# haoningwu3639/StoryGen

Measured on AMD Instinct MI355X. Metric: UNet denoising steps/sec @512x512, 3 prior-frame ctx, bs=1, higher is better.
Workload: dtype f16; 1 GPU; BASELINE configs[1]: StoryGen denoising loop, 512x512 (64x64x4 latent), R=3 prior frames, CFG batch 3, DDIM, SD-1.5 UNet + attn3 (909M params, synthetic fp16 weights); stage=multi-image-condition, samples_per_gpu=1, parallelism=dp1 (one sample per GPU, final all-gather), hipgraph=True, dedup_identical_reference_samples=True, overlap_ref_pass_of_next_step=True, ref_ahead=1, warmup_run=5, split_graphs=False, stream_priority=False, ref_pass_on_cus=0, ref_pass_eager=False, paired_gemm_launches=True, paired_text_image_attention=False, groupnorm_stats_from_epilogues=True, fp16_block_stream=False

## Files before the change

storygen_amd/csrc/attention.hip:

```cpp
#include "attention_kernel.h"
#include <float.h>

using namespace sgattn;


static int attn_params(const sg_attn_desc* d, AttnParams& p, const char* who) {
    SG_REQUIRE(d != nullptr, "%s: null descriptor", who);
    SG_REQUIRE(d->q && d->k && d->vt && d->o, "%s: null q/k/vt/o", who);
    SG_REQUIRE(d->B > 0 && d->H > 0 && d->Nq > 0 && d->Nk > 0, "%s: bad shape", who);
    if (d->D != 40 && d->D != 80 && d->D != 160)
        return sg_set_error(SG_EUNSUP, "%s: head dim %d not in {40, 80, 160}", who, d->D);
    SG_REQUIRE(d->Nq <= (1 << 30) && d->Nk <= (1 << 30), "%s: Nq and Nk must not exceed 2^30", who);
    SG_REQUIRE(d->scale > 0.f && d->scale <= FLT_MAX, "%s: scale must be finite and > 0", who);
    SG_REQUIRE(d->kv_batches >= 0 && d->kv_batches <= d->B, "%s: kv_batches must be in [0, B]", who);
    SG_REQUIRE(d->kv_batches == 0 || 2 * (int64_t)d->kv_batches >= d->B, "%s: kv_batches must be 0 or at least B / 2", who);
    SG_REQUIRE(d->ldq % 8 == 0 && d->ldk % 8 == 0 && d->ldvt % 8 == 0 && d->ldo % 4 == 0, "%s: row strides", who);
    SG_REQUIRE(d->bsq % 8 == 0 && d->bsk % 8 == 0 && d->bsvt % 8 == 0 && d->bso % 4 == 0, "%s: batch strides", who);
    SG_REQUIRE(sg_aligned16(d->q) && sg_aligned16(d->k) && sg_aligned16(d->vt) && sg_aligned16(d->o), "%s: 16-byte alignment", who);
    const int64_t hd = (int64_t)d->H * d->D;
    SG_REQUIRE(d->ldq >= hd && d->ldk >= hd && d->ldo >= hd, "%s: token stride smaller than H*D", who);
    SG_REQUIRE(d->ldvt >= ((d->Nk + 7) & ~7), "%s: ldvt must cover Nk rounded up to 8 keys", who);
    SG_REQUIRE((int64_t)d->D * d->ldvt < (1ll << 31), "%s: VT head slab too large for 32-bit offsets", who);
    SG_REQUIRE(d->ldk < (1ll << 25), "%s: K tile (64 ldk) too large for 32-bit offsets", who);
    p = AttnParams{};
// ... 29 lines not shown
    if (lse) return attn_plan_grid(pl, d, SG_ATTN_LSE, 4, 3, who);
    const bool big = attn_big(d);
    const SgOptions& opt = sg_options();
    if (d->D == 40) {
        if (big && opt.attn_d40_general) return attn_plan_grid(pl, d, SG_ATTN_GENERAL, 4, 3, who);
        if (big && opt.attn_lean) return attn_plan_grid(pl, d, SG_ATTN_LEAN, 4, 3, who);
        return attn_plan_grid(pl, d, opt.attn_d40_loop == 1 ? SG_ATTN_SHARED_BODY : SG_ATTN_D40_LOOP, big ? 4 : 2, big ? 3 : 2, who);
    }
    if (d->D == 160 && opt.attn_d160 == 4 && d->Nq <= 256 && d->Nk > KVBLK && (long)sg_cdiv(d->Nq, 32) * d->H * d->B <= 256)
        return attn_plan_grid(pl, d, SG_ATTN_KSPLIT, 4, 1, who);
    return attn_plan_grid(pl, d, SG_ATTN_GENERAL, 4, 3, who);
}

static int attn_launch(const AttnParams& p, int D, const sg_attn_plan& pl, hipStream_t st) {
    const bool big = pl.waves == 4;
    switch (pl.family) {
    case SG_ATTN_LSE:
        if (D == 40) launch_attn<40, 4, 3, true, false, true>(p, st);
        else if (D == 80) launch_attn<80, 4, 3, true>(p, st);
        else launch_attn<160, 4, 3, true>(p, st);
        return SG_OK;
    case SG_ATTN_D40_LOOP: big ? launch_attn_d40<4, 3>(p, st) : launch_attn_d40<2, 2>(p, st); return SG_OK;
    case SG_ATTN_SHARED_BODY: big ? launch_attn<40, 4, 3>(p, st) : launch_attn<40, 2, 2>(p, st); return SG_OK;
    case SG_ATTN_LEAN: launch_attn<40, 4, 3, false, true>(p, st); return SG_OK;
    case SG_ATTN_KSPLIT: launch_attn_ksplit<160, 4>(p, st); return SG_OK;
    case SG_ATTN_GENERAL:
        if (D == 40) launch_attn<40, 4, 3, false, false, true>(p, st);
        else if (D == 80) launch_attn<80, 4, 3>(p, st);
        else launch_attn<160, 4, 3>(p, st);
        return SG_OK;
    }
    return sg_set_error(SG_EINVAL, "attention: internal: no kernel for plan family %d", pl.family);
}

static int attn_fwd(const sg_attn_desc* d, float* lse2, sg_stream_t stream) {
    const char* who = lse2 ? "sg_attn_fwd_lse_f16" : "sg_attn_fwd_f16";
    AttnParams p;
    sg_attn_plan pl;
    if (int rc = attn_params(d, p, "sg_attn_fwd_f16")) return rc;
    if (int rc = attn_plan(d, lse2 != nullptr, pl, "sg_attn_fwd_f16")) return rc;
    p.lse2 = lse2;
    if (int rc = attn_launch(p, d->D, pl, (hipStream_t)stream)) return rc;
    SG_CHECK_LAUNCH(who);
    return SG_OK;
}

extern "C" int sg_attn_fwd_f16(const sg_attn_desc* d, sg_stream_t stream) { return attn_fwd(d, nullptr, stream); }

extern "C" int sg_attn_fwd_plan(const sg_attn_desc* d, int32_t lse, sg_attn_plan* out) {
    SG_REQUIRE(out != nullptr, "sg_attn_fwd_plan: null plan");
    AttnParams p;
    if (int rc = attn_params(d, p, "sg_attn_fwd_plan")) return rc;
    return attn_plan(d, lse != 0, *out, "sg_attn_fwd_plan");
}

static int attn_pair_plan(const sg_attn_desc* d0, const sg_attn_desc* d1, sg_attn_pair_plan& pr, const char* who) {
    const SgOptions& opt = sg_options();
    const bool same = d0->D == d1->D && d0->B == d1->B && d0->H == d1->H && d0->Nq == d1->Nq;
    const bool defaults = !(d0->D == 40 && opt.attn_d40_loop == 1);
    pr = sg_attn_pair_plan{};
    if (!same || !defaults) {
        if (int rc = attn_plan(d0, false, pr.p0, who)) return rc;
        return attn_plan(d1, false, pr.p1, who);
    }
    const bool big = d0->D != 40 || attn_big(d0);
    const int family = d0->D == 40 ? SG_ATTN_D40_LOOP : SG_ATTN_GENERAL;
    if (int rc = attn_plan_grid(pr.p0, d0, family, big ? 4 : 2, big ? 3 : 2, who)) return rc;
    pr.p1 = pr.p0;
    SG_REQUIRE((int64_t)pr.p0.workgroups * 2 < (1ll << 31), "%s: the shared grid does not fit", who);
    pr.shared = 1;
    pr.first = d0->Nk >= d1->Nk ? 0 : 1;
    pr.workgroups = 2 * pr.p0.workgroups;
    return SG_OK;
}
// ... 39 lines not shown
```

storygen_amd/csrc/attention_kernel.h:

```cpp
#pragma once
#include "common.h"
#include <stdlib.h>
#include <type_traits>

namespace sgattn {


constexpr int KVBLK = 64;
constexpr float RESCALE_THR = 6.0f;

struct AttnParams {
    const f16* q; long ldq, bsq;
    const f16* k; long ldk, bsk;
    const f16* vt; long ldvt, bsvt;
    f16* o; long ldo, bso;
    int B, H, Nq, Nk, kv_batches, nqb;
    const f16* k2; long bsk2; const f16* vt2; long bsvt2; int Nk2, kv2;
    float scale_log2;
    float* lse2;
};

__device__ __forceinline__ void glds16(const f16* g, char* lds_wave_base) {
    __builtin_amdgcn_global_load_lds((const __attribute__((address_space(1))) void*)g,
                                     (__attribute__((address_space(3))) void*)lds_wave_base, 16, 0, 0);
// ... 4 lines not shown
}

template <int D>
__device__ __forceinline__ int kswz(int row) {
    return D == 40 ? 0 : (D == 80 ? ((row >> 3) & 1) : ((row >> 2) & 3));
}

constexpr int F40_KPAD = 2688;
constexpr int F40_ONES = 128;

template <int D, int NIMG>
constexpr int attn_smem_bytes() {
    return D == 40 ? F40_KPAD + NIMG * (KVBLK * D * 2 + D * 128 + F40_ONES) : NIMG * (KVBLK * D * 2 + D * 128) + (D % 16 == 0 ? 0 : 16);
}

template <int D, int NW, int S, bool LSE, bool LEAN = false, bool GENERAL = false, bool KSPLIT = false>
__device__ __forceinline__ void attn_fwd_body(const AttnParams& p, char* smem, const int block, const int nblocks) {
    constexpr int SUB = KSPLIT ? NW : 1;
    constexpr bool F40 = D == 40 && !GENERAL;
    constexpr int DC = D / 8;
    constexpr int NDK = (D + 15) / 16;
    constexpr int DT = (D + 31) / 32;
    constexpr int KROW = D * 2;
    constexpr int K_BYTES = KVBLK * KROW;
    constexpr int V_BYTES = D * 128;
    constexpr int K_SEG = K_BYTES / 1024, V_SEG = V_BYTES / 1024, NSEG = K_SEG + V_SEG;
    constexpr int TSTAGE = K_BYTES + V_BYTES + (F40 ? F40_ONES : 0);
    constexpr int STAGE = SUB * TSTAGE;
    constexpr int RING0 = F40 ? F40_KPAD : 0;
    constexpr int MAXL = (NSEG + NW - 1) / NW;
    constexpr int REM = NSEG % NW;
    static_assert(KSPLIT ? (S == 1 && !LSE && !(D == 40 && !GENERAL)) : (S == 2 || S == 3), "2 or 3 stages; key split: one stage of NW tiles");
    static_assert(!KSPLIT || NW * (8 + DT * 64) * 64 <= S * SUB * (KVBLK * D * 2 + D * 128), "the merge images of the waves fit the dead ring");
    static_assert((S - 1) * MAXL < 64, "vmcnt is a 6-bit counter");
    static_assert(RING0 + S * STAGE + (F40 || D % 16 == 0 ? 0 : 16) <= attn_smem_bytes<D, S * SUB>(), "LDS size");
    static_assert(!F40 || (32 * KROW + 16 <= F40_KPAD && F40_KPAD % 128 == 0), "K pad constants of both 32-key blocks");

    const int t = threadIdx.x, lane = t & 63, l31 = lane & 31, hi = lane >> 5;
    const int wave = __builtin_amdgcn_readfirstlane(t >> 6);
    const int work = xcd_remap(block, nblocks);
    const int bh = work / p.nqb, qb = work - bh * p.nqb;
    const int h = bh / p.B, b = bh - h * p.B;
    const int kvb = b < p.kv_batches ? b : b - (p.B - p.kv_batches);
    const bool short_row = kvb < p.kv2;
    const int Nk = short_row ? p.Nk2 : p.Nk;
    const int q0 = KSPLIT ? qb * 32 : (qb * NW + wave) * 32;
    const f16* Q = p.q + (long)b * p.bsq + (long)h * D;
    const f16* K = (short_row ? p.k2 + (long)kvb * p.bsk2 : p.k + (long)(kvb - p.kv2) * p.bsk) + (long)h * D;
    const f16* VT = (short_row ? p.vt2 + (long)kvb * p.bsvt2 : p.vt + (long)(kvb - p.kv2) * p.bsvt) + (long)h * D * p.ldvt;
// ... 22 lines not shown
            const int s = (g - K_SEG) * 64 + lane;
            const int d = s >> 3, cs = s & 7;
            row = d * (int)p.ldvt;
            col = (cs ^ ((d >> 1) & 7)) * 8;
        }
    };
    unsigned off[MAXL];
#pragma unroll
    for (int i = 0; i < MAXL; ++i) {
        const int g = i * NW + wave;
        int row, col;
        coords(g, row, col);
        off[i] = g < K_SEG ? (unsigned)(row * (int)p.ldk + col) : (unsigned)(row + col);
    }
    const int ntiles = (Nk + KVBLK - 1) / KVBLK;
    auto issue_tile = [&](int tile, char* base) __attribute__((always_inline)) {
        const int key0 = tile * KVBLK;
        if (key0 + KVBLK <= Nk) {
            const f16* Kt = K + (long)key0 * p.ldk;
            const f16* Vt = VT + key0;
#pragma unroll
            for (int i = 0; i < MAXL; ++i) {
                const int g = i * NW + wave;
                const f16* src = (g < K_SEG ? Kt : Vt) + off[i];
                if ((i + 1) * NW <= NSEG || g < NSEG) glds16(src, base + g * 1024);
            }
        } else {
#pragma unroll
            for (int i = 0; i < MAXL; ++i) {
                const int g = i * NW + wave;
                int row, col;
                coords(g, row, col);
                if (g < K_SEG) {
                    const int key = min(key0 + row, Nk - 1);
                    glds16(K + (long)key * p.ldk + col, base + g * 1024);
                } else if (g < NSEG) {
                    const int kc = min(key0 + col, nkp8 - 8);
                    glds16(VT + row + kc, base + g * 1024);
                }
            }
// ... 24 lines not shown

    f32x16 oacc[DT];
#pragma unroll
    for (int i = 0; i < DT; ++i)
#pragma unroll
        for (int r = 0; r < 16; ++r) oacc[i][r] = 0.f;
    float m_run = F40 ? 0.f : -INFINITY;
    float l_run = 0.f;

    const int ngroups = (ntiles + SUB - 1) / SUB;
#pragma unroll
    for (int s = 0; s < S - 1; ++s)
        if (s < ngroups) issue(s, s);

    const int prow = (l31 & ~12) | ((l31 & 4) << 1) | ((l31 & 8) >> 1);
    constexpr bool UNR = D == 40;
    int rt_stage = 0;
    for (int group0 = 0; group0 < ngroups; group0 += (UNR ? S : 1)) {
#pragma unroll
    for (int ustage = 0; ustage < (UNR ? S : 1); ++ustage) {
        const int group = group0 + ustage;
        const int stage = UNR ? ustage : rt_stage;
        if (group < ngroups) {
        if constexpr (KSPLIT) {
            if (group > 0) __builtin_amdgcn_s_barrier();
            issue(group, 0);
            wait_vmcnt<0>();
            __builtin_amdgcn_s_barrier();
        } else {
        if (S == 3 && group + 1 < ngroups) {
// ... 1 lines not shown
            else wait_vmcnt<(MAXL > 1 ? MAXL - 1 : 0)>();
        } else {
            wait_vmcnt<0>();
        }
        __builtin_amdgcn_s_barrier();
        if (group + S - 1 < ngroups) {
            int st = stage + S - 1;
            if (st >= S) st -= S;
            issue(group + S - 1, st);
        }
        }
#pragma unroll
      for (int subi = 0; subi < 1; ++subi) {
        const int sub = KSPLIT ? wave : subi;
        const int tile = group * SUB + sub;
        if (tile < ntiles) {
        const char* sK = smem + RING0 + stage * STAGE + sub * TSTAGE;
        const char* sV = sK + K_BYTES;

        f32x16 s[2];
        const f32x16 zero16 = {0.f, 0.f, 0.f, 0.f, 0.f, 0.f, 0.f, 0.f, 0.f, 0.f, 0.f, 0.f, 0.f, 0.f, 0.f, 0.f};
        constexpr bool KBATCH = NDK <= 5;
        if constexpr (KBATCH) {
            f16x8 kf[2][NDK];
            if constexpr (F40) {
                const char* k01 = sK + prow * KROW + hi * 16;
                const char* k2 = hi ? smem : sK + prow * KROW + 64;
#pragma unroll
                for (int kb = 0; kb < 2; ++kb) {
                    kf[kb][0] = *reinterpret_cast<const f16x8*>(k01 + kb * 32 * KROW);
                    kf[kb][1] = *reinterpret_cast<const f16x8*>(k01 + kb * 32 * KROW + 32);
                    kf[kb][2] = *reinterpret_cast<const f16x8*>(k2 + kb * 32 * KROW);
                }
            } else {
#pragma unroll
                for (int kb = 0; kb < 2; ++kb) {
                    const int row = kb * 32 + prow;
                    const char* krow = sK + row * KROW;
                    const int sw = kswz<D>(row);
#pragma unroll
                    for (int st = 0; st < NDK; ++st)
                        kf[kb][st] = *reinterpret_cast<const f16x8*>(krow + (((st * 2 + hi) ^ sw) << 4));
                }
            }
            __builtin_amdgcn_sched_barrier(0);
#pragma unroll
            for (int kb = 0; kb < 2; ++kb)
#pragma unroll
                for (int st = 0; st < NDK; ++st)
                    s[kb] = __builtin_amdgcn_mfma_f32_32x32x16_f16(kf[kb][st], qf[st], st == 0 ? zero16 : s[kb], 0, 0, 0);
        } else {
            const char* krow0 = sK + prow * KROW;
            const char* krow1 = sK + (32 + prow) * KROW;
            const int sw0 = kswz<D>(prow), sw1 = kswz<D>(32 + prow);
            f16x8 k0 = *reinterpret_cast<const f16x8*>(krow0 + ((hi ^ sw0) << 4));
            f16x8 k1 = *reinterpret_cast<const f16x8*>(krow1 + ((hi ^ sw1) << 4));
#pragma unroll
            for (int st = 0; st < NDK; ++st) {
                f16x8 k0n = k0, k1n = k1;
                if (st + 1 < NDK) {
                    k0n = *reinterpret_cast<const f16x8*>(krow0 + ((((st + 1) * 2 + hi) ^ sw0) << 4));
                    k1n = *reinterpret_cast<const f16x8*>(krow1 + ((((st + 1) * 2 + hi) ^ sw1) << 4));
                }
                __builtin_amdgcn_sched_barrier(0);
                s[0] = __builtin_amdgcn_mfma_f32_32x32x16_f16(k0, qf[st], st == 0 ? zero16 : s[0], 0, 0, 0);
                s[1] = __builtin_amdgcn_mfma_f32_32x32x16_f16(k1, qf[st], st == 0 ? zero16 : s[1], 0, 0, 0);
                k0 = k0n; k1 = k1n;
            }
        }
        constexpr bool VPRE = DT <= 3 && !LEAN;
        constexpr int DLAST = F40 ? D : D - 1;
        f16x8 vf[VPRE ? 4 : 1][DT];
        if constexpr (VPRE) {
#pragma unroll
            for (int ks = 0; ks < 4; ++ks)
#pragma unroll
                for (int i = 0; i < DT; ++i) {
                    const int d = min(i * 32 + l31, DLAST);
                    vf[ks][i] = *reinterpret_cast<const f16x8*>(sV + d * 128 + (((ks * 2 + hi) ^ ((d >> 1) & 7)) << 4));
                }
        }
        if ((tile + 1) * KVBLK > Nk) {
#pragma unroll
            for (int kb = 0; kb < 2; ++kb)
#pragma unroll
                for (int r = 0; r < 16; ++r) {
                    const int key = tile * KVBLK + kb * 32 + 16 * (r >> 3) + 8 * hi + (r & 7);
                    if (key >= Nk) s[kb][r] = -INFINITY;
                }
        }
        float mx = s[0][0];
#pragma unroll
        for (int kb = 0; kb < 2; ++kb)
#pragma unroll
            for (int r = 0; r < 16; ++r) mx = fmaxf(mx, s[kb][r]);
        if constexpr (F40) {
            mx = fmaxf(mx, __shfl_xor(mx, 32, 64));
            if (tile == 0 || __builtin_amdgcn_ballot_w64(mx > RESCALE_THR) != 0) {
                float m_new = m_run + (tile == 0 ? mx : fmaxf(mx, 0.f));
                m_new = fminf(fmaxf(m_new, -60000.f), 60000.f);
                const f16 mh = (f16)m_new;
                const f16 ml = (f16)(m_new - (float)mh);
                m_new = (float)mh + (float)ml;
                const float delta = m_new - m_run;
                if (tile != 0) {
                    const float alpha = __builtin_amdgcn_exp2f(-delta);
#pragma unroll
                    for (int i = 0; i < DT; ++i)
#pragma unroll
                        for (int r = 0; r < 16; ++r) oacc[i][r] *= alpha;
                }
#pragma unroll
                for (int kb = 0; kb < 2; ++kb)
#pragma unroll
                    for (int r = 0; r < 16; ++r) s[kb][r] -= delta;
                m_run = m_new;
                if (hi) { qf[NDK - 1][0] = -mh; qf[NDK - 1][1] = -ml; }
            }
#pragma unroll
            for (int kb = 0; kb < 2; ++kb)
#pragma unroll
                for (int r = 0; r < 16; ++r) s[kb][r] = __builtin_amdgcn_exp2f(s[kb][r]);
        } else {
            mx = fmaxf(mx, __shfl_xor(mx, 32, 64)) * p.scale_log2;
            if (__builtin_amdgcn_ballot_w64(mx - m_run > RESCALE_THR) != 0) {
                const float m_new = fmaxf(m_run, mx);
                const float alpha = __builtin_amdgcn_exp2f(m_run - m_new);
                m_run = m_new;
                l_run *= alpha;
#pragma unroll
                for (int i = 0; i < DT; ++i)
#pragma unroll
                    for (int r = 0; r < 16; ++r) oacc[i][r] *= alpha;
            }
            float psum = 0.f;
#pragma unroll
            for (int kb = 0; kb < 2; ++kb)
#pragma unroll
                for (int r = 0; r < 16; ++r) {
                    const float e = __builtin_amdgcn_exp2f(fmaf(s[kb][r], p.scale_log2, -m_run));
                    s[kb][r] = e;
                    psum += e;
                }
            l_run += psum;
        }

        if constexpr (!VPRE) {
#pragma unroll
            for (int i = 0; i < DT; ++i) {
                const int d = min(i * 32 + l31, DLAST);
                vf[0][i] = *reinterpret_cast<const f16x8*>(sV + d * 128 + ((hi ^ ((d >> 1) & 7)) << 4));
            }
        }
#pragma unroll
        for (int ks = 0; ks < 4; ++ks) {
            f16x8 pf;
#pragma unroll
            for (int j = 0; j < 8; ++j) pf[j] = (f16)s[ks >> 1][(ks & 1) * 8 + j];
            f16x8 vn[VPRE ? 1 : DT];
            if constexpr (!VPRE) {
                if (ks + 1 < 4) {
#pragma unroll
                    for (int i = 0; i < DT; ++i) {
                        const int d = min(i * 32 + l31, DLAST);
                        vn[i] = *reinterpret_cast<const f16x8*>(sV + d * 128 + ((((ks + 1) * 2 + hi) ^ ((d >> 1) & 7)) << 4));
                    }
                }
                __builtin_amdgcn_sched_barrier(0);
            }
#pragma unroll
            for (int i = 0; i < DT; ++i)
                oacc[i] = __builtin_amdgcn_mfma_f32_32x32x16_f16(vf[VPRE ? ks : 0][i], pf, oacc[i], 0, 0, 0);
            if constexpr (!VPRE) {
                if (ks + 1 < 4) {
#pragma unroll
                    for (int i = 0; i < DT; ++i) vf[0][i] = vn[i];
                }
            }
        }
        }
      }
        }
        if (!UNR && ++rt_stage == S) rt_stage = 0;
    }
    }

    float l_tot;
    if constexpr (F40) l_tot = oacc[DT - 1][4];
    else l_tot = l_run + __shfl_xor(l_run, 32, 64);
    if constexpr (KSPLIT) {
        constexpr int IMG = (8 + DT * 64) * 64;
        __builtin_amdgcn_s_barrier();
        if (wave > 0) {
            float* img = reinterpret_cast<float*>(smem + (wave - 1) * IMG);
            img[lane] = m_run;
            img[64 + lane] = l_tot;
#pragma unroll
            for (int i = 0; i < DT; ++i)
// ... 332 lines not shown
template <int NW, int S>
void launch_attn_d40(const AttnParams& p0, hipStream_t st) {
    AttnParams p = p0;
    p.nqb = sg_cdiv(p.Nq, 32 * NW);
    hipLaunchKernelGGL((attn_d40_kernel<NW, S>), dim3(p.nqb * p.H * p.B), dim3(64 * NW), 0, st, p);
}

template <int NW, int S>
void launch_attn_d40_pair(const AttnParams& a0, const AttnParams& b0, hipStream_t st) {
    AttnParams a = a0, b = b0;
    a.nqb = sg_cdiv(a.Nq, 32 * NW); b.nqb = sg_cdiv(b.Nq, 32 * NW);
    const int na = a.nqb * a.H * a.B, nb = b.nqb * b.H * b.B;
    hipLaunchKernelGGL((attn_d40_pair_kernel<NW, S>), dim3(na + nb), dim3(64 * NW), 0, st, a, b, na);
}

template <int D, int NW, int S, bool LSE = false, bool LEAN = false, bool GENERAL = false>
__global__ __launch_bounds__(64 * NW) void attn_fwd_kernel(const AttnParams p) {
    __shared__ __attribute__((aligned(16))) char smem[attn_smem_bytes<D, S>()];
    attn_fwd_body<D, NW, S, LSE, LEAN, GENERAL>(p, smem, (int)blockIdx.x, (int)gridDim.x);
}

template <int D, int NW>
__global__ __launch_bounds__(64 * NW) void attn_fwd_ksplit_kernel(const AttnParams p) {
    __shared__ __attribute__((aligned(16))) char smem[attn_smem_bytes<D, NW>()];
    attn_fwd_body<D, NW, 1, false, false, false, true>(p, smem, (int)blockIdx.x, (int)gridDim.x);
}

template <int D, int NW>
void launch_attn_ksplit(const AttnParams& p0, hipStream_t st) {
    AttnParams p = p0;
    p.nqb = sg_cdiv(p.Nq, 32);
    hipLaunchKernelGGL((attn_fwd_ksplit_kernel<D, NW>), dim3(p.nqb * p.H * p.B), dim3(64 * NW), 0, st, p);
}

template <int D, int NW, int S>
__global__ __launch_bounds__(64 * NW) void attn_fwd_pair_kernel(const AttnParams a, const AttnParams b, const int na) {
    __shared__ __attribute__((aligned(16))) char smem[attn_smem_bytes<D, S>()];
    if ((int)blockIdx.x < na) attn_fwd_body<D, NW, S, false>(a, smem, (int)blockIdx.x, na);
    else attn_fwd_body<D, NW, S, false>(b, smem, (int)blockIdx.x - na, (int)gridDim.x - na);
}

template <int D, int NW, int S, bool LSE = false, bool LEAN = false, bool GENERAL = false>
void launch_attn(const AttnParams& p0, hipStream_t st) {
    AttnParams p = p0;
    p.nqb = sg_cdiv(p.Nq, 32 * NW);
    hipLaunchKernelGGL((attn_fwd_kernel<D, NW, S, LSE, LEAN, GENERAL>), dim3(p.nqb * p.H * p.B), dim3(64 * NW), 0, st, p);
}

template <int D, int NW, int S>
void launch_attn_pair(const AttnParams& a0, const AttnParams& b0, hipStream_t st) {
    AttnParams a = a0, b = b0;
    a.nqb = sg_cdiv(a.Nq, 32 * NW); b.nqb = sg_cdiv(b.Nq, 32 * NW);
    const int na = a.nqb * a.H * a.B, nb = b.nqb * b.H * b.B;
    hipLaunchKernelGGL((attn_fwd_pair_kernel<D, NW, S>), dim3(na + nb), dim3(64 * NW), 0, st, a, b, na);
}


}
```

storygen_amd/csrc/common.h:

```cpp
#pragma once
#include <hip/hip_runtime.h>
#include <stdint.h>
#include <stdio.h>
#include <stdarg.h>

#include "../../include/storygen_hip.h"

typedef _Float16 f16;
typedef f16 f16x2 __attribute__((ext_vector_type(2)));
typedef f16 f16x4 __attribute__((ext_vector_type(4)));
typedef f16 f16x8 __attribute__((ext_vector_type(8)));
typedef float f32x4 __attribute__((ext_vector_type(4)));
typedef float f32x16 __attribute__((ext_vector_type(16)));

int sg_set_error(int code, const char* fmt, ...);

#define SG_REQUIRE(cond, ...)                                   \
    do {                                                        \
        if (!(cond)) return sg_set_error(SG_EINVAL, __VA_ARGS__); \
    } while (0)

#define SG_CHECK_LAUNCH(name)                                                                  \
    do {                                                                                       \
        hipError_t e__ = hipGetLastError();                                                    \
// ... 7 lines not shown
    int tile_m = 0, tile_n = 0;
    int no_pipe = 0, no_split = 0;
    int no_nmajor = 0;
    int pipe_stages = 3;
    int lat_tiles = 640;
    int lat_min_kt = 8, lat_max_kt = 64;
    int lat_stages = 4;
    int lat_mask = 62;
    int big_m = 0, big_bm = 0, big_bn = 0;
    int fat_m = 0;
    int lat_wide = 0, lat_wide_m = 256;
    int attn_d160 = 4;
    int attn_lean = 0;
    int attn_d40_general = 0;
    int attn_d40_loop = 0;
    int gn_no_fused = 0, gn_wide = 1;
    int gn_fused_nt = 1024;
    int gn_chunks = 0;
    int ff_variant = 3;
    long gn_fused_max = -1;
};
SgOptions& sg_options();

__device__ __forceinline__ uint4 ldg16(const void* p) { return *reinterpret_cast<const uint4*>(p); }
__device__ __forceinline__ void stg16(void* p, uint4 v) { *reinterpret_cast<uint4*>(p) = v; }

union H8 {
    uint4 u;
    f16x8 v;
    f16 h[8];
// ... 47 lines not shown
```

storygen_amd/csrc/misc.hip:

```cpp
#include "common.h"
#include <string.h>

static thread_local char g_err[512] = "";

SgOptions& sg_options() {
    static SgOptions o;
    return o;
}

extern "C" int sg_debug_set_option(const char* name, int64_t value) {
    if (!name) return sg_set_error(SG_EINVAL, "sg_debug_set_option: null name");
    SgOptions& o = sg_options();
    struct Entry { const char* n; int* p; };
    const Entry table[] = {{"tile_m", &o.tile_m}, {"tile_n", &o.tile_n}, {"no_pipe", &o.no_pipe}, {"no_split", &o.no_split},
                           {"no_nmajor", &o.no_nmajor}, {"attn_d160", &o.attn_d160}, {"gn_no_fused", &o.gn_no_fused},
                           {"gn_wide", &o.gn_wide}, {"attn_lean", &o.attn_lean}, {"attn_d40_general", &o.attn_d40_general}, {"attn_d40_loop", &o.attn_d40_loop},
                           {"gn_fused_nt", &o.gn_fused_nt}, {"pipe_stages", &o.pipe_stages}, {"ff_variant", &o.ff_variant},
                           {"gn_chunks", &o.gn_chunks}, {"lat_tiles", &o.lat_tiles}, {"lat_min_kt", &o.lat_min_kt},
                           {"lat_max_kt", &o.lat_max_kt}, {"lat_stages", &o.lat_stages}, {"lat_wide", &o.lat_wide}, {"lat_mask", &o.lat_mask}, {"lat_wide_m", &o.lat_wide_m}, {"fat_m", &o.fat_m}, {"big_m", &o.big_m}, {"big_bm", &o.big_bm}, {"big_bn", &o.big_bn}};
    for (const Entry& e : table)
        if (strcmp(e.n, name) == 0) {
            if (e.p == &o.attn_d160 && value != 3 && value != 4)
                return sg_set_error(SG_EINVAL, "sg_debug_set_option: attn_d160 must be 3 (query split) or 4 (key split where it applies)");
            *e.p = (int)value;
            return SG_OK;
        }
    if (strcmp(name, "gn_fused_max") == 0) {
        o.gn_fused_max = (long)value;
        return SG_OK;
    }
    if (strcmp(name, "reset") == 0) {
// ... 438 lines not shown
```

storygen_amd/ops.py:

```python
from __future__ import annotations

import ctypes as C
from typing import Optional

import torch

from . import _lib
from ._lib import AttnDesc, AttnPairPlan, AttnPlan, ConvDesc, FfDesc, GemmDesc, GnPlan, GroupNormDesc, check

lib = _lib.load()

EPI_LINEAR = 0
EPI_GEGLU = 1
F_OUT_F32, F_RES1_F32, F_RES2_F32 = 1, 2, 4

TILE_TABLE = {}
TUNE_SINK = None


def _apply_tile(d, tile, split_k, sig, mn):
    if tile is not None:
        d.tile_m, d.tile_n = tile[0], tile[1]
        if len(tile) > 2:
            d.tile_waves = tile[2]
# ... 1182 lines not shown
    with _timed("attention_bwd", 8.0 * d.B * d.H * d.Nq * d.Nk * d.D, f"dkv B{d.B} H{d.H} Nq{d.Nq} Nk{d.Nk} D{d.D}"):
        check(lib.sg_attn_bwd_dkv_f16(C.byref(d), _stream()), "sg_attn_bwd_dkv_f16")
    return dkt, dvt


def debug_set_tile(bm: int = 0, bn: int = 0, no_pipe: bool = False) -> None:
    check(lib.sg_debug_set_tile(bm, bn, int(no_pipe)), "sg_debug_set_tile")


def debug_set_option(name: str, value: int) -> None:
    check(lib.sg_debug_set_option(name.encode(), int(value)), "sg_debug_set_option")


_ENV_OPTIONS = {"SG_NO_NMAJOR": "no_nmajor", "SG_NO_PIPE": "no_pipe", "SG_NO_SPLIT": "no_split",
                "SG_ATTN_D160": "attn_d160",
                "SG_FF_VARIANT": "ff_variant", "SG_PIPE_STAGES": "pipe_stages", "SG_GN_FUSED_NT": "gn_fused_nt", "SG_GN_CHUNKS": "gn_chunks", "SG_ATTN_LEAN": "attn_lean", "SG_ATTN_D40_GENERAL": "attn_d40_general", "SG_ATTN_D40_LOOP": "attn_d40_loop","SG_NO_GN_FUSED": "gn_no_fused", "SG_GN_WIDE": "gn_wide", "SG_GN_FUSED_MAX": "gn_fused_max",
                "SG_LAT_TILES": "lat_tiles", "SG_LAT_MIN_KT": "lat_min_kt", "SG_LAT_MAX_KT": "lat_max_kt", "SG_LAT_STAGES": "lat_stages", "SG_LAT_WIDE": "lat_wide", "SG_LAT_MASK": "lat_mask", "SG_LAT_WIDE_M": "lat_wide_m", "SG_FAT_M": "fat_m", "SG_BIG_M": "big_m", "SG_BIG_BM": "big_bm", "SG_BIG_BN": "big_bn"}


def apply_env_options() -> dict:
    import os
    done = {}
    for var, name in _ENV_OPTIONS.items():
        if os.environ.get(var, "") != "":
            debug_set_option(name, int(os.environ[var]))
            done[name] = int(os.environ[var])
    if os.environ.get("SG_TILE"):
        bm, bn = (int(v) for v in os.environ["SG_TILE"].split(","))
        debug_set_option("tile_m", bm), debug_set_option("tile_n", bn)
        done["tile"] = (bm, bn)
    return done
# ... 18 lines not shown
```

Baseline: 81.52 denoising steps/s.

## Peel first and tail tiles out of the attention key loop for D=80/160

```diff
diff --git a/storygen_amd/csrc/attention.hip b/storygen_amd/csrc/attention.hip
--- a/storygen_amd/csrc/attention.hip
+++ b/storygen_amd/csrc/attention.hip
@@ -67,6 +67,7 @@
 
 static int attn_launch(const AttnParams& p, int D, const sg_attn_plan& pl, hipStream_t st) {
     const bool big = pl.waves == 4;
+    const bool peel = sg_options().attn_tiles_loop != 1;
     switch (pl.family) {
     case SG_ATTN_LSE:
         if (D == 40) launch_attn<40, 4, 3, true, false, true>(p, st);
@@ -76,11 +77,11 @@
     case SG_ATTN_D40_LOOP: big ? launch_attn_d40<4, 3>(p, st) : launch_attn_d40<2, 2>(p, st); return SG_OK;
     case SG_ATTN_SHARED_BODY: big ? launch_attn<40, 4, 3>(p, st) : launch_attn<40, 2, 2>(p, st); return SG_OK;
     case SG_ATTN_LEAN: launch_attn<40, 4, 3, false, true>(p, st); return SG_OK;
-    case SG_ATTN_KSPLIT: launch_attn_ksplit<160, 4>(p, st); return SG_OK;
+    case SG_ATTN_KSPLIT: peel ? launch_attn_ksplit<160, 4, true>(p, st) : launch_attn_ksplit<160, 4, false>(p, st); return SG_OK;
     case SG_ATTN_GENERAL:
         if (D == 40) launch_attn<40, 4, 3, false, false, true>(p, st);
-        else if (D == 80) launch_attn<80, 4, 3>(p, st);
-        else launch_attn<160, 4, 3>(p, st);
+        else if (D == 80) peel ? launch_attn<80, 4, 3, false, false, false, true>(p, st) : launch_attn<80, 4, 3>(p, st);
+        else peel ? launch_attn<160, 4, 3, false, false, false, true>(p, st) : launch_attn<160, 4, 3>(p, st);
         return SG_OK;
     }
     return sg_set_error(SG_EINVAL, "attention: internal: no kernel for plan family %d", pl.family);
@@ -110,7 +111,7 @@
 static int attn_pair_plan(const sg_attn_desc* d0, const sg_attn_desc* d1, sg_attn_pair_plan& pr, const char* who) {
     const SgOptions& opt = sg_options();
     const bool same = d0->D == d1->D && d0->B == d1->B && d0->H == d1->H && d0->Nq == d1->Nq;
-    const bool defaults = !(d0->D == 40 && opt.attn_d40_loop == 1);
+    const bool defaults = !(d0->D == 40 ? opt.attn_d40_loop == 1 : opt.attn_tiles_loop == 1);
     pr = sg_attn_pair_plan{};
     if (!same || !defaults) {
         if (int rc = attn_plan(d0, false, pr.p0, who)) return rc;
diff --git a/storygen_amd/csrc/attention_kernel.h b/storygen_amd/csrc/attention_kernel.h
--- a/storygen_amd/csrc/attention_kernel.h
+++ b/storygen_amd/csrc/attention_kernel.h
@@ -42,7 +42,7 @@
     return D == 40 ? F40_KPAD + NIMG * (KVBLK * D * 2 + D * 128 + F40_ONES) : NIMG * (KVBLK * D * 2 + D * 128) + (D % 16 == 0 ? 0 : 16);
 }
 
-template <int D, int NW, int S, bool LSE, bool LEAN = false, bool GENERAL = false, bool KSPLIT = false>
+template <int D, int NW, int S, bool LSE, bool LEAN = false, bool GENERAL = false, bool KSPLIT = false, bool PEEL = false>
 __device__ __forceinline__ void attn_fwd_body(const AttnParams& p, char* smem, const int block, const int nblocks) {
     constexpr int SUB = KSPLIT ? NW : 1;
     constexpr bool F40 = D == 40 && !GENERAL;
@@ -61,6 +61,7 @@
     static_assert(KSPLIT ? (S == 1 && !LSE && !(D == 40 && !GENERAL)) : (S == 2 || S == 3), "2 or 3 stages; key split: one stage of NW tiles");
     static_assert(!KSPLIT || NW * (8 + DT * 64) * 64 <= S * SUB * (KVBLK * D * 2 + D * 128), "the merge images of the waves fit the dead ring");
     static_assert((S - 1) * MAXL < 64, "vmcnt is a 6-bit counter");
+    static_assert(!PEEL || (!F40 && !LSE && !LEAN && REM == 0), "peeled loop: general softmax, inference, every wave issues MAXL pieces per tile");
     static_assert(RING0 + S * STAGE + (F40 || D % 16 == 0 ? 0 : 16) <= attn_smem_bytes<D, S * SUB>(), "LDS size");
     static_assert(!F40 || (32 * KROW + 16 <= F40_KPAD && F40_KPAD % 128 == 0), "K pad constants of both 32-key blocks");
 
@@ -113,16 +114,26 @@
         off[i] = g < K_SEG ? (unsigned)(row * (int)p.ldk + col) : (unsigned)(row + col);
     }
     const int ntiles = (Nk + KVBLK - 1) / KVBLK;
+    constexpr int IX = K_SEG % NW != 0 ? K_SEG / NW : -1;
+    const bool x_is_k = IX >= 0 && IX * NW + wave < K_SEG;
+    auto issue_full = [&](const f16* Kt, const f16* Vt, const f16* Xt, char* base) __attribute__((always_inline)) {
+#pragma unroll
+        for (int i = 0; i < MAXL; ++i) glds16((i == IX ? Xt : i * NW < K_SEG ? Kt : Vt) + off[i], base + (i * NW + wave) * 1024);
+    };
     auto issue_tile = [&](int tile, char* base) __attribute__((always_inline)) {
         const int key0 = tile * KVBLK;
         if (key0 + KVBLK <= Nk) {
             const f16* Kt = K + (long)key0 * p.ldk;
             const f16* Vt = VT + key0;
-#pragma unroll
-            for (int i = 0; i < MAXL; ++i) {
-                const int g = i * NW + wave;
-                const f16* src = (g < K_SEG ? Kt : Vt) + off[i];
-                if ((i + 1) * NW <= NSEG || g < NSEG) glds16(src, base + g * 1024);
+            if constexpr (PEEL) {
+                issue_full(Kt, Vt, x_is_k ? Kt : Vt, base);
+            } else {
+#pragma unroll
+                for (int i = 0; i < MAXL; ++i) {
+                    const int g = i * NW + wave;
+                    const f16* src = (g < K_SEG ? Kt : Vt) + off[i];
+                    if ((i + 1) * NW <= NSEG || g < NSEG) glds16(src, base + g * 1024);
+                }
             }
         } else {
 #pragma unroll
@@ -177,6 +188,253 @@
         if (s < ngroups) issue(s, s);
 
     const int prow = (l31 & ~12) | ((l31 & 4) << 1) | ((l31 & 8) >> 1);
+
+    auto compute = [&](auto first_, auto mask_, const char* sK, const int tile) __attribute__((always_inline)) {
+        constexpr bool FIRST = decltype(first_)::value, MASK = decltype(mask_)::value;
+        static_assert(!FIRST || !F40, "the fast path tests tile == 0 itself");
+        const char* sV = sK + K_BYTES;
+
+        f32x16 s[2];
+        const f32x16 zero16 = {0.f, 0.f, 0.f, 0.f, 0.f, 0.f, 0.f, 0.f, 0.f, 0.f, 0.f, 0.f, 0.f, 0.f, 0.f, 0.f};
+        constexpr bool KBATCH = NDK <= 5;
+        if constexpr (KBATCH) {
+            f16x8 kf[2][NDK];
+            if constexpr (F40) {
+                const char* k01 = sK + prow * KROW + hi * 16;
+                const char* k2 = hi ? smem : sK + prow * KROW + 64;
+#pragma unroll
+                for (int kb = 0; kb < 2; ++kb) {
+                    kf[kb][0] = *reinterpret_cast<const f16x8*>(k01 + kb * 32 * KROW);
+                    kf[kb][1] = *reinterpret_cast<const f16x8*>(k01 + kb * 32 * KROW + 32);
+                    kf[kb][2] = *reinterpret_cast<const f16x8*>(k2 + kb * 32 * KROW);
+                }
+            } else {
+#pragma unroll
+                for (int kb = 0; kb < 2; ++kb) {
+                    const int row = kb * 32 + prow;
+                    const char* krow = sK + row * KROW;
+                    const int sw = kswz<D>(row);
+#pragma unroll
+                    for (int st = 0; st < NDK; ++st)
+                        kf[kb][st] = *reinterpret_cast<const f16x8*>(krow + (((st * 2 + hi) ^ sw) << 4));
+                }
+            }
+            __builtin_amdgcn_sched_barrier(0);
+#pragma unroll
+            for (int kb = 0; kb < 2; ++kb)
+#pragma unroll
+                for (int st = 0; st < NDK; ++st)
+                    s[kb] = __builtin_amdgcn_mfma_f32_32x32x16_f16(kf[kb][st], qf[st], st == 0 ? zero16 : s[kb], 0, 0, 0);
+        } else {
+            const char* krow0 = sK + prow * KROW;
+            const char* krow1 = sK + (32 + prow) * KROW;
+            const int sw0 = kswz<D>(prow), sw1 = kswz<D>(32 + prow);
+            f16x8 k0 = *reinterpret_cast<const f16x8*>(krow0 + ((hi ^ sw0) << 4));
+            f16x8 k1 = *reinterpret_cast<const f16x8*>(krow1 + ((hi ^ sw1) << 4));
+#pragma unroll
+            for (int st = 0; st < NDK; ++st) {
+                f16x8 k0n = k0, k1n = k1;
+                if (st + 1 < NDK) {
+                    k0n = *reinterpret_cast<const f16x8*>(krow0 + ((((st + 1) * 2 + hi) ^ sw0) << 4));
+                    k1n = *reinterpret_cast<const f16x8*>(krow1 + ((((st + 1) * 2 + hi) ^ sw1) << 4));
+                }
+                __builtin_amdgcn_sched_barrier(0);
+                s[0] = __builtin_amdgcn_mfma_f32_32x32x16_f16(k0, qf[st], st == 0 ? zero16 : s[0], 0, 0, 0);
+                s[1] = __builtin_amdgcn_mfma_f32_32x32x16_f16(k1, qf[st], st == 0 ? zero16 : s[1], 0, 0, 0);
+                k0 = k0n; k1 = k1n;
+            }
+        }
+        constexpr bool VPRE = DT <= 3 && !LEAN;
+        constexpr int DLAST = F40 ? D : D - 1;
+        f16x8 vf[VPRE ? 4 : 1][DT];
+        if constexpr (VPRE) {
+#pragma unroll
+            for (int ks = 0; ks < 4; ++ks)
+#pragma unroll
+                for (int i = 0; i < DT; ++i) {
+                    const int d = min(i * 32 + l31, DLAST);
+                    vf[ks][i] = *reinterpret_cast<const f16x8*>(sV + d * 128 + (((ks * 2 + hi) ^ ((d >> 1) & 7)) << 4));
+                }
+        }
+        if (MASK && (tile + 1) * KVBLK > Nk) {
+#pragma unroll
+            for (int kb = 0; kb < 2; ++kb)
+#pragma unroll
+                for (int r = 0; r < 16; ++r) {
+                    const int key = tile * KVBLK + kb * 32 + 16 * (r >> 3) + 8 * hi + (r & 7);
+                    if (key >= Nk) s[kb][r] = -INFINITY;
+                }
+        }
+        float mx = s[0][0];
+#pragma unroll
+        for (int kb = 0; kb < 2; ++kb)
+#pragma unroll
+            for (int r = 0; r < 16; ++r) mx = fmaxf(mx, s[kb][r]);
+        if constexpr (F40) {
+            mx = fmaxf(mx, __shfl_xor(mx, 32, 64));
+            if (tile == 0 || __builtin_amdgcn_ballot_w64(mx > RESCALE_THR) != 0) {
+                float m_new = m_run + (tile == 0 ? mx : fmaxf(mx, 0.f));
+                m_new = fminf(fmaxf(m_new, -60000.f), 60000.f);
+                const f16 mh = (f16)m_new;
+                const f16 ml = (f16)(m_new - (float)mh);
+                m_new = (float)mh + (float)ml;
+                const float delta = m_new - m_run;
+                if (tile != 0) {
+                    const float alpha = __builtin_amdgcn_exp2f(-delta);
+#pragma unroll
+                    for (int i = 0; i < DT; ++i)
+#pragma unroll
+                        for (int r = 0; r < 16; ++r) oacc[i][r] *= alpha;
+                }
+#pragma unroll
+                for (int kb = 0; kb < 2; ++kb)
+#pragma unroll
+                    for (int r = 0; r < 16; ++r) s[kb][r] -= delta;
+                m_run = m_new;
+                if (hi) { qf[NDK - 1][0] = -mh; qf[NDK - 1][1] = -ml; }
+            }
+#pragma unroll
+            for (int kb = 0; kb < 2; ++kb)
+#pragma unroll
+                for (int r = 0; r < 16; ++r) s[kb][r] = __builtin_amdgcn_exp2f(s[kb][r]);
+        } else {
+            mx = fmaxf(mx, __shfl_xor(mx, 32, 64)) * p.scale_log2;
+            if constexpr (FIRST) {
+                m_run = mx;
+            } else if (__builtin_amdgcn_ballot_w64(mx - m_run > RESCALE_THR) != 0) {
+                const float m_new = fmaxf(m_run, mx);
+                const float alpha = __builtin_amdgcn_exp2f(m_run - m_new);
+                m_run = m_new;
+                l_run *= alpha;
+#pragma unroll
+                for (int i = 0; i < DT; ++i)
+#pragma unroll
+                    for (int r = 0; r < 16; ++r) oacc[i][r] *= alpha;
+            }
+            float psum = 0.f;
+#pragma unroll
+            for (int kb = 0; kb < 2; ++kb)
+#pragma unroll
+                for (int r = 0; r < 16; ++r) {
+                    const float e = __builtin_amdgcn_exp2f(fmaf(s[kb][r], p.scale_log2, -m_run));
+                    s[kb][r] = e;
+                    psum += e;
+                }
+            l_run += psum;
+        }
+
+        if constexpr (!VPRE) {
+#pragma unroll
+            for (int i = 0; i < DT; ++i) {
+                const int d = min(i * 32 + l31, DLAST);
+                vf[0][i] = *reinterpret_cast<const f16x8*>(sV + d * 128 + ((hi ^ ((d >> 1) & 7)) << 4));
+            }
+        }
+#pragma unroll
+        for (int ks = 0; ks < 4; ++ks) {
+            f16x8 pf;
+#pragma unroll
+            for (int j = 0; j < 8; ++j) pf[j] = (f16)s[ks >> 1][(ks & 1) * 8 + j];
+            f16x8 vn[VPRE ? 1 : DT];
+            if constexpr (!VPRE) {
+                if (ks + 1 < 4) {
+#pragma unroll
+                    for (int i = 0; i < DT; ++i) {
+                        const int d = min(i * 32 + l31, DLAST);
+                        vn[i] = *reinterpret_cast<const f16x8*>(sV + d * 128 + ((((ks + 1) * 2 + hi) ^ ((d >> 1) & 7)) << 4));
+                    }
+                }
+                __builtin_amdgcn_sched_barrier(0);
+            }
+#pragma unroll
+            for (int i = 0; i < DT; ++i)
+                oacc[i] = __builtin_amdgcn_mfma_f32_32x32x16_f16(vf[VPRE ? ks : 0][i], pf, oacc[i], 0, 0, 0);
+            if constexpr (!VPRE) {
+                if (ks + 1 < 4) {
+#pragma unroll
+                    for (int i = 0; i < DT; ++i) vf[0][i] = vn[i];
+                }
+            }
+        }
+    };
+    using T = std::true_type;
+    using F = std::false_type;
+    char* const ring = smem + RING0;
+
+    if constexpr (PEEL) {
+        const int nfull = Nk / KVBLK;
+        const long kstep = (long)KVBLK * p.ldk;
+        if constexpr (KSPLIT) {
+            issue(0, 0);
+            wait_vmcnt<0>();
+            __builtin_amdgcn_s_barrier();
+            if (wave < ntiles) compute(T{}, T{}, ring + wave * TSTAGE, wave);
+            int group = 1;
+            const f16* Kn = K + SUB * kstep;
+            const f16* Vn = VT + SUB * KVBLK;
+            for (; (group + 1) * SUB <= nfull; ++group) {
+                __builtin_amdgcn_s_barrier();
+#pragma unroll
+                for (int sub = 0; sub < SUB; ++sub) {
+                    const f16* Kt = Kn + sub * kstep;
+                    const f16* Vt = Vn + sub * KVBLK;
+                    issue_full(Kt, Vt, x_is_k ? Kt : Vt, ring + sub * TSTAGE);
+                }
+                Kn += SUB * kstep; Vn += SUB * KVBLK;
+                wait_vmcnt<0>();
+                __builtin_amdgcn_s_barrier();
+                compute(F{}, F{}, ring + wave * TSTAGE, 0);
+            }
+            for (; group < ngroups; ++group) {
+                __builtin_amdgcn_s_barrier();
+                issue(group, 0);
+                wait_vmcnt<0>();
+                __builtin_amdgcn_s_barrier();
+                const int tile = group * SUB + wave;
+                if (tile < ntiles) compute(F{}, T{}, ring + wave * TSTAGE, tile);
+            }
+        } else {
+            if (S == 3 && 1 < ntiles) wait_vmcnt<MAXL>();
+            else wait_vmcnt<0>();
+            __builtin_amdgcn_s_barrier();
+            if (S - 1 < ntiles) issue_tile(S - 1, ring + (S - 1) * STAGE);
+            compute(T{}, T{}, ring, 0);
+
+            int tile = 1;
+            const f16* Kn = K + S * kstep;
+            const f16* Vn = VT + S * KVBLK;
+            const f16* Xn = x_is_k ? Kn : Vn;
+            const long xstep = x_is_k ? kstep : (long)KVBLK;
+            for (; tile + 2 * S - 2 < nfull; tile += S) {
+                auto step = [&](auto stage_) __attribute__((always_inline)) {
+                    constexpr int STG = decltype(stage_)::value;
+                    wait_vmcnt<(S == 3 ? MAXL : 0)>();
+                    __builtin_amdgcn_s_barrier();
+                    issue_full(Kn, Vn, Xn, ring + ((STG + S - 1) % S) * STAGE);
+                    Kn += kstep; Vn += KVBLK; Xn += xstep;
+                    compute(F{}, F{}, ring + STG * STAGE, 0);
+                };
+                step(std::integral_constant<int, 1 % S>{});
+                step(std::integral_constant<int, 2 % S>{});
+                if constexpr (S == 3) step(std::integral_constant<int, 0>{});
+            }
+            for (; tile < ntiles; tile += S) {
+                auto step = [&](auto stage_, const int tl) __attribute__((always_inline)) {
+                    constexpr int STG = decltype(stage_)::value;
+                    if (tl < ntiles) {
+                        if (S == 3 && tl + 1 < ntiles) wait_vmcnt<MAXL>();
+                        else wait_vmcnt<0>();
+                        __builtin_amdgcn_s_barrier();
+                        if (tl + S - 1 < ntiles) issue_tile(tl + S - 1, ring + ((STG + S - 1) % S) * STAGE);
+                        compute(F{}, T{}, ring + STG * STAGE, tl);
+                    }
+                };
+                step(std::integral_constant<int, 1 % S>{}, tile);
+                step(std::integral_constant<int, 2 % S>{}, tile + 1);
+                if constexpr (S == 3) step(std::integral_constant<int, 0>{}, tile + 2);
+            }
+        }
+    } else {
     constexpr bool UNR = D == 40;
     int rt_stage = 0;
     for (int group0 = 0; group0 < ngroups; group0 += (UNR ? S : 1)) {
@@ -208,174 +466,11 @@
       for (int subi = 0; subi < 1; ++subi) {
         const int sub = KSPLIT ? wave : subi;
         const int tile = group * SUB + sub;
-        if (tile < ntiles) {
-        const char* sK = smem + RING0 + stage * STAGE + sub * TSTAGE;
-        const char* sV = sK + K_BYTES;
-
-        f32x16 s[2];
-        const f32x16 zero16 = {0.f, 0.f, 0.f, 0.f, 0.f, 0.f, 0.f, 0.f, 0.f, 0.f, 0.f, 0.f, 0.f, 0.f, 0.f, 0.f};
-        constexpr bool KBATCH = NDK <= 5;
-        if constexpr (KBATCH) {
-            f16x8 kf[2][NDK];
-            if constexpr (F40) {
-                const char* k01 = sK + prow * KROW + hi * 16;
-                const char* k2 = hi ? smem : sK + prow * KROW + 64;
-#pragma unroll
-                for (int kb = 0; kb < 2; ++kb) {
-                    kf[kb][0] = *reinterpret_cast<const f16x8*>(k01 + kb * 32 * KROW);
-                    kf[kb][1] = *reinterpret_cast<const f16x8*>(k01 + kb * 32 * KROW + 32);
-                    kf[kb][2] = *reinterpret_cast<const f16x8*>(k2 + kb * 32 * KROW);
-                }
-            } else {
-#pragma unroll
-                for (int kb = 0; kb < 2; ++kb) {
-                    const int row = kb * 32 + prow;
-                    const char* krow = sK + row * KROW;
-                    const int sw = kswz<D>(row);
-#pragma unroll
-                    for (int st = 0; st < NDK; ++st)
-                        kf[kb][st] = *reinterpret_cast<const f16x8*>(krow + (((st * 2 + hi) ^ sw) << 4));
-                }
-            }
-            __builtin_amdgcn_sched_barrier(0);
-#pragma unroll
-            for (int kb = 0; kb < 2; ++kb)
-#pragma unroll
-                for (int st = 0; st < NDK; ++st)
-                    s[kb] = __builtin_amdgcn_mfma_f32_32x32x16_f16(kf[kb][st], qf[st], st == 0 ? zero16 : s[kb], 0, 0, 0);
-        } else {
-            const char* krow0 = sK + prow * KROW;
-            const char* krow1 = sK + (32 + prow) * KROW;
-            const int sw0 = kswz<D>(prow), sw1 = kswz<D>(32 + prow);
-            f16x8 k0 = *reinterpret_cast<const f16x8*>(krow0 + ((hi ^ sw0) << 4));
-            f16x8 k1 = *reinterpret_cast<const f16x8*>(krow1 + ((hi ^ sw1) << 4));
-#pragma unroll
-            for (int st = 0; st < NDK; ++st) {
-                f16x8 k0n = k0, k1n = k1;
-                if (st + 1 < NDK) {
-                    k0n = *reinterpret_cast<const f16x8*>(krow0 + ((((st + 1) * 2 + hi) ^ sw0) << 4));
-                    k1n = *reinterpret_cast<const f16x8*>(krow1 + ((((st + 1) * 2 + hi) ^ sw1) << 4));
-                }
-                __builtin_amdgcn_sched_barrier(0);
-                s[0] = __builtin_amdgcn_mfma_f32_32x32x16_f16(k0, qf[st], st == 0 ? zero16 : s[0], 0, 0, 0);
-                s[1] = __builtin_amdgcn_mfma_f32_32x32x16_f16(k1, qf[st], st == 0 ? zero16 : s[1], 0, 0, 0);
-                k0 = k0n; k1 = k1n;
-            }
-        }
-        constexpr bool VPRE = DT <= 3 && !LEAN;
-        constexpr int DLAST = F40 ? D : D - 1;
-        f16x8 vf[VPRE ? 4 : 1][DT];
-        if constexpr (VPRE) {
-#pragma unroll
-            for (int ks = 0; ks < 4; ++ks)
-#pragma unroll
-                for (int i = 0; i < DT; ++i) {
-                    const int d = min(i * 32 + l31, DLAST);
-                    vf[ks][i] = *reinterpret_cast<const f16x8*>(sV + d * 128 + (((ks * 2 + hi) ^ ((d >> 1) & 7)) << 4));
-                }
-        }
-        if ((tile + 1) * KVBLK > Nk) {
-#pragma unroll
-            for (int kb = 0; kb < 2; ++kb)
-#pragma unroll
-                for (int r = 0; r < 16; ++r) {
-                    const int key = tile * KVBLK + kb * 32 + 16 * (r >> 3) + 8 * hi + (r & 7);
-                    if (key >= Nk) s[kb][r] = -INFINITY;
-                }
-        }
-        float mx = s[0][0];
-#pragma unroll
-        for (int kb = 0; kb < 2; ++kb)
-#pragma unroll
-            for (int r = 0; r < 16; ++r) mx = fmaxf(mx, s[kb][r]);
-        if constexpr (F40) {
-            mx = fmaxf(mx, __shfl_xor(mx, 32, 64));
-            if (tile == 0 || __builtin_amdgcn_ballot_w64(mx > RESCALE_THR) != 0) {
-                float m_new = m_run + (tile == 0 ? mx : fmaxf(mx, 0.f));
-                m_new = fminf(fmaxf(m_new, -60000.f), 60000.f);
-                const f16 mh = (f16)m_new;
-                const f16 ml = (f16)(m_new - (float)mh);
-                m_new = (float)mh + (float)ml;
-                const float delta = m_new - m_run;
-                if (tile != 0) {
-                    const float alpha = __builtin_amdgcn_exp2f(-delta);
-#pragma unroll
-                    for (int i = 0; i < DT; ++i)
-#pragma unroll
-                        for (int r = 0; r < 16; ++r) oacc[i][r] *= alpha;
-                }
-#pragma unroll
-                for (int kb = 0; kb < 2; ++kb)
-#pragma unroll
-                    for (int r = 0; r < 16; ++r) s[kb][r] -= delta;
-                m_run = m_new;
-                if (hi) { qf[NDK - 1][0] = -mh; qf[NDK - 1][1] = -ml; }
-            }
-#pragma unroll
-            for (int kb = 0; kb < 2; ++kb)
-#pragma unroll
-                for (int r = 0; r < 16; ++r) s[kb][r] = __builtin_amdgcn_exp2f(s[kb][r]);
-        } else {
-            mx = fmaxf(mx, __shfl_xor(mx, 32, 64)) * p.scale_log2;
-            if (__builtin_amdgcn_ballot_w64(mx - m_run > RESCALE_THR) != 0) {
-                const float m_new = fmaxf(m_run, mx);
-                const float alpha = __builtin_amdgcn_exp2f(m_run - m_new);
-                m_run = m_new;
-                l_run *= alpha;
-#pragma unroll
-                for (int i = 0; i < DT; ++i)
-#pragma unroll
-                    for (int r = 0; r < 16; ++r) oacc[i][r] *= alpha;
-            }
-            float psum = 0.f;
-#pragma unroll
-            for (int kb = 0; kb < 2; ++kb)
-#pragma unroll
-                for (int r = 0; r < 16; ++r) {
-                    const float e = __builtin_amdgcn_exp2f(fmaf(s[kb][r], p.scale_log2, -m_run));
-                    s[kb][r] = e;
-                    psum += e;
-                }
-            l_run += psum;
-        }
-
-        if constexpr (!VPRE) {
-#pragma unroll
-            for (int i = 0; i < DT; ++i) {
-                const int d = min(i * 32 + l31, DLAST);
-                vf[0][i] = *reinterpret_cast<const f16x8*>(sV + d * 128 + ((hi ^ ((d >> 1) & 7)) << 4));
-            }
-        }
-#pragma unroll
-        for (int ks = 0; ks < 4; ++ks) {
-            f16x8 pf;
-#pragma unroll
-            for (int j = 0; j < 8; ++j) pf[j] = (f16)s[ks >> 1][(ks & 1) * 8 + j];
-            f16x8 vn[VPRE ? 1 : DT];
-            if constexpr (!VPRE) {
-                if (ks + 1 < 4) {
-#pragma unroll
-                    for (int i = 0; i < DT; ++i) {
-                        const int d = min(i * 32 + l31, DLAST);
-                        vn[i] = *reinterpret_cast<const f16x8*>(sV + d * 128 + ((((ks + 1) * 2 + hi) ^ ((d >> 1) & 7)) << 4));
-                    }
-                }
-                __builtin_amdgcn_sched_barrier(0);
-            }
-#pragma unroll
-            for (int i = 0; i < DT; ++i)
-                oacc[i] = __builtin_amdgcn_mfma_f32_32x32x16_f16(vf[VPRE ? ks : 0][i], pf, oacc[i], 0, 0, 0);
-            if constexpr (!VPRE) {
-                if (ks + 1 < 4) {
-#pragma unroll
-                    for (int i = 0; i < DT; ++i) vf[0][i] = vn[i];
-                }
-            }
-        }
-        }
+        if (tile < ntiles) compute(F{}, T{}, ring + stage * STAGE + sub * TSTAGE, tile);
       }
         }
         if (!UNR && ++rt_stage == S) rt_stage = 0;
+    }
     }
     }
 
@@ -738,37 +833,37 @@
     hipLaunchKernelGGL((attn_d40_pair_kernel<NW, S>), dim3(na + nb), dim3(64 * NW), 0, st, a, b, na);
 }
 
-template <int D, int NW, int S, bool LSE = false, bool LEAN = false, bool GENERAL = false>
+template <int D, int NW, int S, bool LSE = false, bool LEAN = false, bool GENERAL = false, bool PEEL = false>
 __global__ __launch_bounds__(64 * NW) void attn_fwd_kernel(const AttnParams p) {
     __shared__ __attribute__((aligned(16))) char smem[attn_smem_bytes<D, S>()];
-    attn_fwd_body<D, NW, S, LSE, LEAN, GENERAL>(p, smem, (int)blockIdx.x, (int)gridDim.x);
-}
-
-template <int D, int NW>
+    attn_fwd_body<D, NW, S, LSE, LEAN, GENERAL, false, PEEL>(p, smem, (int)blockIdx.x, (int)gridDim.x);
+}
+
+template <int D, int NW, bool PEEL>
 __global__ __launch_bounds__(64 * NW) void attn_fwd_ksplit_kernel(const AttnParams p) {
     __shared__ __attribute__((aligned(16))) char smem[attn_smem_bytes<D, NW>()];
-    attn_fwd_body<D, NW, 1, false, false, false, true>(p, smem, (int)blockIdx.x, (int)gridDim.x);
-}
-
-template <int D, int NW>
+    attn_fwd_body<D, NW, 1, false, false, false, true, PEEL>(p, smem, (int)blockIdx.x, (int)gridDim.x);
+}
+
+template <int D, int NW, bool PEEL>
 void launch_attn_ksplit(const AttnParams& p0, hipStream_t st) {
     AttnParams p = p0;
     p.nqb = sg_cdiv(p.Nq, 32);
-    hipLaunchKernelGGL((attn_fwd_ksplit_kernel<D, NW>), dim3(p.nqb * p.H * p.B), dim3(64 * NW), 0, st, p);
+    hipLaunchKernelGGL((attn_fwd_ksplit_kernel<D, NW, PEEL>), dim3(p.nqb * p.H * p.B), dim3(64 * NW), 0, st, p);
 }
 
 template <int D, int NW, int S>
 __global__ __launch_bounds__(64 * NW) void attn_fwd_pair_kernel(const AttnParams a, const AttnParams b, const int na) {
     __shared__ __attribute__((aligned(16))) char smem[attn_smem_bytes<D, S>()];
-    if ((int)blockIdx.x < na) attn_fwd_body<D, NW, S, false>(a, smem, (int)blockIdx.x, na);
-    else attn_fwd_body<D, NW, S, false>(b, smem, (int)blockIdx.x - na, (int)gridDim.x - na);
-}
-
-template <int D, int NW, int S, bool LSE = false, bool LEAN = false, bool GENERAL = false>
+    if ((int)blockIdx.x < na) attn_fwd_body<D, NW, S, false, false, false, false, true>(a, smem, (int)blockIdx.x, na);
+    else attn_fwd_body<D, NW, S, false, false, false, false, true>(b, smem, (int)blockIdx.x - na, (int)gridDim.x - na);
+}
+
+template <int D, int NW, int S, bool LSE = false, bool LEAN = false, bool GENERAL = false, bool PEEL = false>
 void launch_attn(const AttnParams& p0, hipStream_t st) {
     AttnParams p = p0;
     p.nqb = sg_cdiv(p.Nq, 32 * NW);
-    hipLaunchKernelGGL((attn_fwd_kernel<D, NW, S, LSE, LEAN, GENERAL>), dim3(p.nqb * p.H * p.B), dim3(64 * NW), 0, st, p);
+    hipLaunchKernelGGL((attn_fwd_kernel<D, NW, S, LSE, LEAN, GENERAL, PEEL>), dim3(p.nqb * p.H * p.B), dim3(64 * NW), 0, st, p);
 }
 
 template <int D, int NW, int S>
diff --git a/storygen_amd/csrc/common.h b/storygen_amd/csrc/common.h
--- a/storygen_amd/csrc/common.h
+++ b/storygen_amd/csrc/common.h
@@ -45,6 +45,7 @@
     int attn_lean = 0;
     int attn_d40_general = 0;
     int attn_d40_loop = 0;
+    int attn_tiles_loop = 0;
     int gn_no_fused = 0, gn_wide = 1;
     int gn_fused_nt = 1024;
     int gn_chunks = 0;
diff --git a/storygen_amd/csrc/misc.hip b/storygen_amd/csrc/misc.hip
--- a/storygen_amd/csrc/misc.hip
+++ b/storygen_amd/csrc/misc.hip
@@ -14,7 +14,7 @@
     struct Entry { const char* n; int* p; };
     const Entry table[] = {{"tile_m", &o.tile_m}, {"tile_n", &o.tile_n}, {"no_pipe", &o.no_pipe}, {"no_split", &o.no_split},
                            {"no_nmajor", &o.no_nmajor}, {"attn_d160", &o.attn_d160}, {"gn_no_fused", &o.gn_no_fused},
-                           {"gn_wide", &o.gn_wide}, {"attn_lean", &o.attn_lean}, {"attn_d40_general", &o.attn_d40_general}, {"attn_d40_loop", &o.attn_d40_loop},
+                           {"gn_wide", &o.gn_wide}, {"attn_lean", &o.attn_lean}, {"attn_d40_general", &o.attn_d40_general}, {"attn_d40_loop", &o.attn_d40_loop}, {"attn_tiles_loop", &o.attn_tiles_loop},
                            {"gn_fused_nt", &o.gn_fused_nt}, {"pipe_stages", &o.pipe_stages}, {"ff_variant", &o.ff_variant},
                            {"gn_chunks", &o.gn_chunks}, {"lat_tiles", &o.lat_tiles}, {"lat_min_kt", &o.lat_min_kt},
                            {"lat_max_kt", &o.lat_max_kt}, {"lat_stages", &o.lat_stages}, {"lat_wide", &o.lat_wide}, {"lat_mask", &o.lat_mask}, {"lat_wide_m", &o.lat_wide_m}, {"fat_m", &o.fat_m}, {"big_m", &o.big_m}, {"big_bm", &o.big_bm}, {"big_bn", &o.big_bn}};
diff --git a/storygen_amd/ops.py b/storygen_amd/ops.py
--- a/storygen_amd/ops.py
+++ b/storygen_amd/ops.py
@@ -1220,7 +1220,7 @@
 
 _ENV_OPTIONS = {"SG_NO_NMAJOR": "no_nmajor", "SG_NO_PIPE": "no_pipe", "SG_NO_SPLIT": "no_split",
                 "SG_ATTN_D160": "attn_d160",
-                "SG_FF_VARIANT": "ff_variant", "SG_PIPE_STAGES": "pipe_stages", "SG_GN_FUSED_NT": "gn_fused_nt", "SG_GN_CHUNKS": "gn_chunks", "SG_ATTN_LEAN": "attn_lean", "SG_ATTN_D40_GENERAL": "attn_d40_general", "SG_ATTN_D40_LOOP": "attn_d40_loop","SG_NO_GN_FUSED": "gn_no_fused", "SG_GN_WIDE": "gn_wide", "SG_GN_FUSED_MAX": "gn_fused_max",
+                "SG_FF_VARIANT": "ff_variant", "SG_PIPE_STAGES": "pipe_stages", "SG_GN_FUSED_NT": "gn_fused_nt", "SG_GN_CHUNKS": "gn_chunks", "SG_ATTN_LEAN": "attn_lean", "SG_ATTN_D40_GENERAL": "attn_d40_general", "SG_ATTN_D40_LOOP": "attn_d40_loop", "SG_ATTN_TILES_LOOP": "attn_tiles_loop","SG_NO_GN_FUSED": "gn_no_fused", "SG_GN_WIDE": "gn_wide", "SG_GN_FUSED_MAX": "gn_fused_max",
                 "SG_LAT_TILES": "lat_tiles", "SG_LAT_MIN_KT": "lat_min_kt", "SG_LAT_MAX_KT": "lat_max_kt", "SG_LAT_STAGES": "lat_stages", "SG_LAT_WIDE": "lat_wide", "SG_LAT_MASK": "lat_mask", "SG_LAT_WIDE_M": "lat_wide_m", "SG_FAT_M": "fat_m", "SG_BIG_M": "big_m", "SG_BIG_BM": "big_bm", "SG_BIG_BN": "big_bn"}
 
 
```

Result: no change. 81.56 denoising steps/s, median of 3 (+0.0%).
